# fritzsedlazeck/Sniffles

Measured on NVIDIA H100. Metric: aligned long-read Gbp/s through lead->cluster->consensus, higher is better.
Workload: dtype int32

## Files before the change

sniffles_b200/csrc/api.cu:

```cuda
#include <algorithm>
#include <climits>
#include <cstdio>
#include <cstdlib>
#include <cstring>
#include <string>
#include <vector>
#include <dlfcn.h>
#include <omp.h>

#include "common.cuh"
#include "prims.cuh"
#include "extract.cuh"
#include "cluster.cuh"
#include "consensus.cuh"
#include "poa.cuh"
#include "combine.cuh"
#include "ingest.cuh"
#include "bgzf_write.cuh"

template <bool Pinned> struct Buf {
    void* p = nullptr; size_t cap = 0;
    Buf() = default;
    Buf(const Buf&) = delete; Buf& operator=(const Buf&) = delete;
    ~Buf() { release(); }
// ... 213 lines not shown
    for (int i = 0; i <= MAX_TIMINGS; ++i) cudaEventDestroy(ctx->ev[i]);
    cudaEventDestroy(ctx->ev_b); cudaEventDestroy(ctx->ev_mid); cudaEventDestroy(ctx->ev_fork); cudaEventDestroy(ctx->ev_join);
    cudaStreamDestroy(ctx->st_side); cudaStreamDestroy(ctx->st_copy); cudaStreamDestroy(ctx->st);
    delete ctx;
}

const char* snfb_last_error(snfb_ctx* ctx) { return ctx ? ctx->err.c_str() : "null context"; }

int snfb_set_config(snfb_ctx* ctx, const snfb_config* cfg) {
    if (!ctx || !cfg) return 1;
    ctx->force_no_cuts = false;
    if (cfg->consensus_kmer_len != 6) return fail(ctx, "consensus_kmer_len must be 6 (the reference fixes it, config.py:550)");
    if (cfg->cluster_binsize <= 0 || cfg->cluster_resplit_binsize <= 0 || cfg->coverage_binsize <= 0) return fail(ctx, "bin sizes must be positive");
    ctx->cfg = *cfg; ctx->have_cfg = true; ctx->stage_a_done = ctx->stage_b_done = ctx->stage_c_done = false; return 0;
}

static bool c16_offsets(const snfb_rec* rec_in, uint64_t n_rec, const uint32_t* cigar32, std::vector<uint64_t>& off) {
    off.assign(n_rec + 1, 0);
    const uint8_t* raw = reinterpret_cast<const uint8_t*>(cigar32);
    bool bad = false;
    #pragma omp parallel for schedule(static) reduction(|| : bad)
    for (long long i = 0; i < (long long)n_rec; ++i) {
        long long ref; int b = 0;
        const uint32_t w = ingest::c16_convert<1>(raw, 4ull * rec_in[i].cigar_off, rec_in[i].n_cigar, nullptr, 0, 0, &ref, &b);
        bad = bad || b; off[i + 1] = (w + 7) & ~7ull;
    }
    if (bad) return false;
    for (uint64_t i = 0; i < n_rec; ++i) off[i + 1] += off[i];
    return true;
}
static void c16_fill(const snfb_rec* rec_in, uint64_t n_rec, const uint32_t* cigar32, const std::vector<uint64_t>& off, snfb_rec* rec_out, uint16_t* out16, uint32_t evt_min) {
    const uint8_t* raw = reinterpret_cast<const uint8_t*>(cigar32);
    #pragma omp parallel for schedule(static)
    for (long long i = 0; i < (long long)n_rec; ++i) {
        uint16_t* dst = out16 + off[i]; const uint64_t span = off[i + 1] - off[i];
        long long ref; int bad = 0;
        const uint64_t k = ingest::c16_convert<1>(raw, 4ull * rec_in[i].cigar_off, rec_in[i].n_cigar, dst, evt_min, 0, &ref, &bad);
        if (k < span) memset(dst + k, 0, 2 * (span - k));
        snfb_rec r = rec_in[i]; r.n_cigar = (uint32_t)k; r.cigar_off = off[i];
        rec_out[i] = r;
    }
    memset(out16 + off[n_rec], 0, 16);
}
uint64_t snfb_pack_cigar16(const snfb_rec* rec_in, uint64_t n_rec, const uint32_t* cigar32, snfb_rec* rec_out, uint16_t* out16, uint64_t out_cap, uint32_t evt_min) {
    if (n_rec && (!rec_in || !cigar32)) return UINT64_MAX;
    if (evt_min == 0) evt_min = SNFB_CIGAR16_EVT_MIN;
    std::vector<uint64_t> off;
    if (!c16_offsets(rec_in, n_rec, cigar32, off)) return UINT64_MAX;
    const uint64_t total = off[n_rec] + 8;
    if (!out16) return total;
    if (!rec_out || out_cap < total) return UINT64_MAX;
    c16_fill(rec_in, n_rec, cigar32, off, rec_out, out16, evt_min);
    return total;
}

__global__ void k_validate(const snfb_rec* __restrict__ rec, uint32_t n_rec, uint32_t n_task, uint64_t n_cigar, uint64_t n_var, uint64_t n_seq, int check_seq, DevCounters* ctr) {
    const uint32_t i = blockIdx.x * blockDim.x + threadIdx.x; if (i >= n_rec) return;
    const snfb_rec r = rec[i];
    bool bad = r.task < 0 || (uint32_t)r.task >= n_task || (r.cigar_off & 7) || r.cigar_off + (uint64_t)r.n_cigar > n_cigar || r.var_off + (uint64_t)r.l_qname + r.sa_len > n_var || r.l_seq < 0;
    if (check_seq && r.l_seq >= 0 && r.seq_off + (uint64_t)((r.l_seq + 1) / 2) > n_seq) bad = true;
    if (bad) atomicAdd(&ctr->bad_records, 1ULL);
}

static int check_tables(snfb_ctx* ctx, const snfb_records* R) {
    for (uint32_t t = 0; t < R->n_task; ++t) {
        const snfb_task& k = R->task[t];
        if (k.tr_n < 0 || k.tr_off < 0 || (uint64_t)k.tr_off + (uint64_t)k.tr_n > R->n_tr) return fail(ctx, "task table: tandem-repeat range outside tr[]");
        if (R->n_contig && (k.contig < 0 || (uint32_t)k.contig >= R->n_contig)) return fail(ctx, "task table: contig index out of range");
        if (k.contig_len < 0 || k.start > k.end) return fail(ctx, "task table: bad region");
        if ((long long)k.contig_len >= ((long long)1 << 26) * (long long)(ctx->have_cfg ? ctx->cfg.cluster_binsize : 100)) return fail(ctx, "contig too long for the bin field of the sort key (contig_len / cluster_binsize must stay below 2^26)");
    }
    if (R->n_mask && R->mask && R->mask_task_off) {
        for (uint32_t t = 0; t < R->n_task; ++t) if (R->mask_task_off[t] > R->mask_task_off[t + 1] || R->mask_task_off[t + 1] > R->n_mask) return fail(ctx, "mask_task_off must be non-decreasing and end at n_mask");
    }
    return 0;
}
static int upload_tables(snfb_ctx* ctx, const snfb_records* R) {
    ctx->tasks.assign(R->task, R->task + R->n_task);
    if (ctx->b_task.ensure(sizeof(snfb_task) * R->n_task) || ctx->b_contig.ensure(sizeof(snfb_contig) * (R->n_contig + 1)) || ctx->b_tr.ensure(8 * ((size_t)R->n_tr + 1)) || ctx->b_trp.ensure(4 * ((size_t)R->n_tr + 1)))
        return fail(ctx, "out of device memory for the task tables");
    CUDA_TRY(cudaMemcpyAsync(ctx->b_task.p, R->task, sizeof(snfb_task) * R->n_task, cudaMemcpyHostToDevice, ctx->st));
    if (R->n_contig) CUDA_TRY(cudaMemcpyAsync(ctx->b_contig.p, R->contig, sizeof(snfb_contig) * R->n_contig, cudaMemcpyHostToDevice, ctx->st));
    if (R->n_tr) {
        std::vector<int32_t> pm(R->n_tr);
        for (uint32_t t = 0; t < R->n_task; ++t) { int32_t m = INT32_MIN; for (int k = 0; k < R->task[t].tr_n; ++k) { const int idx = R->task[t].tr_off + k; if (R->tr[2 * idx + 1] > m) m = R->tr[2 * idx + 1]; pm[idx] = m; } }
        CUDA_TRY(cudaMemcpyAsync(ctx->b_tr.p, R->tr, 8 * (size_t)R->n_tr, cudaMemcpyHostToDevice, ctx->st));
        CUDA_TRY(cudaMemcpyAsync(ctx->b_trp.p, pm.data(), 4 * (size_t)R->n_tr, cudaMemcpyHostToDevice, ctx->st));
        CUDA_TRY(cudaStreamSynchronize(ctx->st));
    }
    ctx->n_mask = (R->mask && R->mask_task_off) ? R->n_mask : 0;
    if (ctx->n_mask) {
        std::vector<uint32_t> mt(ctx->n_mask);
        for (uint32_t t = 0; t < R->n_task; ++t) for (uint32_t m = R->mask_task_off[t]; m < R->mask_task_off[t + 1] && m < ctx->n_mask; ++m) mt[m] = t;
        if (ctx->b_mask.ensure(8 * (size_t)ctx->n_mask) || ctx->b_mask_off.ensure(4 * ((size_t)R->n_task + 1)) || ctx->b_mask_task.ensure(4 * (size_t)ctx->n_mask)) return fail(ctx, "out of device memory (N mask)");
        CUDA_TRY(cudaMemcpyAsync(ctx->b_mask.p, R->mask, 8 * (size_t)ctx->n_mask, cudaMemcpyHostToDevice, ctx->st));
        CUDA_TRY(cudaMemcpyAsync(ctx->b_mask_off.p, R->mask_task_off, 4 * ((size_t)R->n_task + 1), cudaMemcpyHostToDevice, ctx->st));
        CUDA_TRY(cudaMemcpyAsync(ctx->b_mask_task.p, mt.data(), 4 * (size_t)ctx->n_mask, cudaMemcpyHostToDevice, ctx->st));
        CUDA_TRY(cudaStreamSynchronize(ctx->st));
    }
    return 0;
}

int snfb_load_records(snfb_ctx* ctx, const snfb_records* R) {
    if (!ctx || !R) return 1;
    cudaSetDevice(ctx->device);
    ctx->loaded = false; ctx->stage_a_done = ctx->stage_b_done = ctx->stage_c_done = false; ctx->force_no_cuts = false;
    if (R->n_task == 0 || R->n_task > 65535) return fail(ctx, "n_task must be in 1..65535");
    if (R->n_rec >= (1ull << 28)) return fail(ctx, "too many records in one block (2^28)");
    if (!R->task || (R->n_rec && (!R->rec || !R->cigar))) return fail(ctx, "null table in the record block");
    if (check_tables(ctx, R)) return 1;
    ctx->n_rec = R->n_rec; ctx->n_cigar = R->n_cigar; ctx->n_var = R->n_var; ctx->n_seq = R->n_seq;
    ctx->n_task = R->n_task; ctx->n_contig = R->n_contig; ctx->n_tr = R->n_tr; ctx->on_device = R->on_device == SNFB_MEM_DEVICE; ctx->seq_on_demand = R->on_device == SNFB_MEM_HOST_SEQ_ON_DEMAND; ctx->h_seq = ctx->seq_on_demand ? R->seq : nullptr;
    ctx->n_ev = 0;
    const snfb_rec* src_rec = R->rec; const uint16_t* src_cigar = reinterpret_cast<const uint16_t*>(R->cigar); uint64_t n_words = R->n_cigar;
// ... 267 lines not shown
    b.cl_nsub = c.take<uint32_t>(n); b.cl_nvalid = c.take<uint32_t>(n); b.cl_nlead = c.take<uint32_t>(n); b.cl_nrn = c.take<uint32_t>(n); b.cl_cand_base = c.take<uint32_t>(n); b.cl_lead_base = c.take<uint32_t>(n); b.cl_rn_base = c.take<uint32_t>(n);
    ctx->arena_off = c.take<uint32_t>(n);
}
static void carve_c(snfb_ctx* ctx, Carver& c) {
    const Caps& k = ctx->cap; cluster::B& b = ctx->B; consensus::C& cc = ctx->Cc;
    b.cand = c.take<snfb_cand>(k.cand + 1); b.cand_leads = c.take<snfb_lead>(k.cand_lead + 1); b.out_plo = c.take<uint32_t>(k.cand_lead + 1); b.out_pn = c.take<uint32_t>(k.cand_lead + 1);
    b.rnames = c.take<uint64_t>(k.rn + 1); b.rn_off_out = c.take<uint32_t>(k.cand + 2);
    cc.plan_best = c.take<uint32_t>(k.cand + 1); cc.plan_nother = c.take<uint32_t>(k.cand + 1); cc.plan_otot = c.take<uint32_t>(k.cand + 1); cc.alt_len = c.take<uint32_t>(k.cand + 1); cc.scr_len = c.take<uint32_t>(k.cand + 1);
    cc.alt_off = c.take<uint32_t>(k.cand + 1); cc.scr_off = c.take<uint32_t>(k.cand + 1); cc.work_big = c.take<uint32_t>(k.cand + 1); cc.work_small = c.take<uint32_t>(k.cand + 1); cc.work_ctr = c.take<uint32_t>(64);
    cc.items_big = c.take<consensus::C::Item>(k.item + 1); cc.items_small = c.take<consensus::C::Item>(k.item + 1); cc.tiles = c.take<uint2>(k.tile + 1);
    cc.alt = c.take<uint8_t>(k.alt + 64); cc.scr = c.take<uint8_t>(k.scr16 * 16 + 64);
    ctx->seq_req = c.take<consensus::SeqReq>(k.req + 1); ctx->seq_arena = c.take<uint8_t>(k.req16 * 16 + 64);
}
static int ensure_arenas(snfb_ctx* ctx) {
    if (carve(ctx->arena_r, [&](Carver& c) { carve_r(ctx, c); })) return fail(ctx, "out of device memory (per-record arrays)");
    if (carve(ctx->arena_l, [&](Carver& c) { carve_l(ctx, c); })) return fail(ctx, "out of device memory (per-lead arrays)");
    if (carve(ctx->arena_c, [&](Carver& c) { carve_c(ctx, c); })) return fail(ctx, "out of device memory (candidate / consensus arrays)");
    return 0;
}

static void bind_inputs(snfb_ctx* ctx) {
    cluster::B& b = ctx->B;
    b.leads = ctx->leads; b.rec = ctx->d_rec; b.task = ctx->b_task.as<snfb_task>(); b.contig = ctx->b_contig.as<snfb_contig>();
    b.tr = ctx->n_tr ? ctx->b_tr.as<int32_t>() : nullptr; b.tr_pmax = ctx->b_trp.as<int32_t>();
    b.rec_pos = ctx->rec_pos; b.rec_end = ctx->rec_end; b.rec_flags = ctx->rec_flags; b.rec_nm = ctx->rec_nm; b.rec_nlead = ctx->rec_nlead; b.rec_lead_off = ctx->rec_lead_off;
    b.task_first = ctx->task_first; b.task_last = ctx->task_last; b.task_maxspan = ctx->task_span;
    b.mask = ctx->n_mask ? ctx->b_mask.as<int32_t>() : nullptr; b.mask_task_off = ctx->n_mask ? ctx->b_mask_off.as<uint32_t>() : nullptr;
    b.n_task = ctx->n_task; b.n_bound = ctx->cap.lead; b.ctr = ctx->b_ctr.as<DevCounters>(); b.cfg = ctx->cfg;
    b.cut_gap = ctx->force_no_cuts ? INT_MAX : cluster::break_gap(ctx->cfg);
    b.cand_cap = ctx->cap.cand; b.cand_lead_cap = ctx->cap.cand_lead; b.rn_cap = ctx->cap.rn;
    consensus::C& c = ctx->Cc;
    c.cand = b.cand; c.cand_rw = b.cand; c.cand_leads = b.cand_leads; c.out_plo = b.out_plo; c.out_pn = b.out_pn; c.ord = b.ord; c.kleads = b.kleads; c.rec = ctx->d_rec; c.seq = ctx->d_seq; c.arena_off = nullptr;
    c.cand_cap = ctx->cap.cand; c.ctr = b.ctr; c.cfg = ctx->cfg; c.item_cap = ctx->cap.item; c.tile_cap = ctx->cap.tile; c.alt_cap = ctx->cap.alt; c.scr_cap16 = ctx->cap.scr16;
}

static int enqueue_stage_a(snfb_ctx* ctx) {
    const uint64_t nrec = ctx->n_rec; const uint32_t nt = ctx->n_task; const snfb_config& cf = ctx->cfg; cluster::B& b = ctx->B;
    DevCounters* ctr = b.ctr; cudaStream_t st = ctx->st;
    CUDA_TRY(cudaMemsetAsync(ctr, 0, sizeof(DevCounters), st));
    CUDA_TRY(cudaMemsetAsync(ctx->task_first, 0, 4 * nt, st)); CUDA_TRY(cudaMemsetAsync(ctx->task_last, 0, 4 * nt, st));
    CUDA_TRY(cudaMemsetAsync(ctx->task_reads, 0, 4 * nt, st)); CUDA_TRY(cudaMemsetAsync(ctx->task_cov, 0, 8 * nt, st)); CUDA_TRY(cudaMemsetAsync(ctx->task_span, 0, 4 * nt, st));
    CUDA_TRY(cudaMemsetAsync(ctx->task_nm, 0, 8 * nt, st));
    extract::WalkParams S{};
    S.scan = ctx->scanrec; S.n_rec = (uint32_t)nrec; S.cigar = ctx->d_cigar; S.task = b.task;
    S.rec_end = ctx->rec_end; S.rec_nlead = ctx->rec_nlead; S.rec_big = ctx->rec_big;
    S.ev = ctx->ev_buf; S.ev_cap = ctx->cap.lead; S.n_ev = &ctr->n_ev; S.ctr = ctr; S.minsv = cf.minsvlen_screen;
    if (evt_need(ctx) < ctx->evt_min) {
        if (ctx->on_device) return fail(ctx, "the device-resident CIGAR16 arena was packed with a larger event length than the configuration needs: repack with snfb_pack_cigar16(evt_min)");
        launch(ctx->launches, extract::k_reflag, NUM_SMS * 8, 256, 0, st, const_cast<uint16_t*>(ctx->d_cigar), ctx->n_cigar, evt_need(ctx));
        ctx->evt_min = evt_need(ctx);
    }
    mark(ctx, "k_rec_index");
    if (nrec) {
        launch(ctx->launches, k_validate, (unsigned)((nrec + 255) / 256), 256, 0, st, ctx->d_rec, (uint32_t)nrec, nt, ctx->n_cigar, ctx->n_var, ctx->n_seq, ctx->seq_on_demand ? 0 : 1, ctr);
        extract::IndexParams I{};
        I.rec = ctx->d_rec; I.cigar = ctx->d_cigar; I.task = b.task; I.n_rec = (uint32_t)nrec; I.n_task = nt; I.rec_pos = ctx->rec_pos; I.task_first = ctx->task_first; I.task_last = ctx->task_last;
        I.scan = ctx->scanrec; I.clip = ctx->clip; I.rec_end = ctx->rec_end; I.rec_flags = ctx->rec_flags; I.rec_nm = ctx->rec_nm; I.rec_nlead = ctx->rec_nlead; I.ctr = ctr;
        I.mapq_min = cf.mapq; I.alen_min = cf.min_alignment_length; I.excl = cf.exclude_flags; I.want_nm = (cf.qc_nm_measure || cf.phase) ? 1 : 0; I.n_cigar = ctx->n_cigar;
        I.sa_list = ctx->sa_list; I.n_sa = &ctr->n_sa;
        launch(ctx->launches, extract::k_rec_index, (unsigned)((nrec + 255) / 256), 256, 0, st, I);
        mark(ctx, "k_scan", 2 * ctx->n_cigar);
        if (nrec >= extract::WALK_WIDE_MIN) launch(ctx->launches, extract::k_cigar_walk<32>, extract::WALK_BLOCKS, extract::WALK_THREADS, 0, st, S);
        else launch(ctx->launches, extract::k_cigar_walk<1>, extract::WALK_BLOCKS, extract::WALK_THREADS, 0, st, S);
        mark(ctx, "k_rec_post");
        extract::PostParams Q{};
        Q.scan = I.scan; Q.clip = I.clip; Q.task = b.task; Q.n_rec = (uint32_t)nrec; Q.rec_end = ctx->rec_end; Q.rec_big = ctx->rec_big; Q.rec_nm = ctx->rec_nm;
        Q.task_reads = ctx->task_reads; Q.task_cov_bp = ctx->task_cov; Q.task_maxspan = ctx->task_span;
        launch(ctx->launches, extract::k_rec_post, (unsigned)((nrec + 255) / 256), 256, 0, st, Q);
        mark(ctx, "k_emit");
        extract::EmitParams E{};
        E.rec = ctx->d_rec; E.clip = ctx->clip; E.var = ctx->d_var; E.ev = S.ev; E.n_ev = S.n_ev; E.ev_cap = ctx->cap.lead;
        E.leads = ctx->leads; E.ctr = ctr; E.maxlen = cf.dev_seq_cache_maxlen; E.detect_large_ins = cf.detect_large_ins; E.longinslen = (double)cf.long_ins_length / 2.0;
        launch(ctx->launches, extract::k_emit, NUM_SMS * 16, 128, 0, st, E);
        mark(ctx, "k_sa");
        extract::SaParams A{};
        A.rec = ctx->d_rec; A.clip = ctx->clip; A.var = ctx->d_var; A.task = b.task; A.contig = b.contig; A.n_contig = ctx->n_contig;
        A.sa_list = ctx->sa_list; A.n_sa = &ctr->n_sa; A.rec_end = ctx->rec_end; A.rec_nlead = ctx->rec_nlead; A.leads = E.leads; A.lead_cap = ctx->cap.lead; A.ctr = ctr; A.cfg = cf; A.seg_scratch = ctx->sa_seg;
        launch(ctx->launches, extract::k_sa, extract::SA_BLOCKS, extract::SA_THREADS, 0, st, A);
        mark(ctx, "k_task_nm");
        const int cpt = (int)((nrec + extract::NM_CHUNK - 1) / extract::NM_CHUNK);
        launch(ctx->launches, extract::k_nm_partial, dim3(cpt, nt), 256, 0, st, ctx->rec_flags, ctx->rec_nm, ctx->task_first, ctx->task_last, ctx->nm_part, ctx->nm_cnt);
        launch(ctx->launches, extract::k_task_nm, nt, 256, 0, st, ctx->task_first, ctx->task_last, ctx->nm_part, ctx->nm_cnt, cpt, ctx->task_nm);
    }
    mark(ctx, "scan_rec_leads");
    prims::exclusive_scan(ctx->launches, ctx->rec_nlead, ctx->rec_lead_off, ctx->scan_tmp_r, nullptr, nrec, &ctr->n_leads, st);
    const unsigned long long nb = b.n_bound; const int g = grid_for(nb, 256);
    mark(ctx, "sort_leads");
    launch(ctx->launches, cluster::k_scatter_keys, g, 256, 0, st, b);
    prims::RadixTemp rt{ ctx->radix_hist, b.scan_tmp };
    bool first = true;
    prims::radix_sort(ctx->launches, b.key0, b.val0, b.key1, b.val1, rt, &ctr->n_leads, nb, cluster::TASK_SHIFT + bits_for(ctx->n_task), &first, st);
    b.skey = first ? b.key0 : b.key1; b.sval = first ? b.val0 : b.val1;
    mark(ctx, "bins");
    launch(ctx->launches, cluster::k_bin_heads, g, 256, 0, st, b);
    prims::exclusive_scan(ctx->launches, b.flag, b.scan, b.scan_tmp, &ctr->n_leads, nb, &ctr->n_bins, st);
    launch(ctx->launches, cluster::k_bin_build, g, 256, 0, st, b);
    launch(ctx->launches, cluster::k_bin_stats, g, 256, 0, st, b);
    mark(ctx, nullptr);
    CUDA_TRY(cudaGetLastError());
    return 0;
}

static int enqueue_stage_b(snfb_ctx* ctx) {
    cluster::B& b = ctx->B; DevCounters* ctr = b.ctr; cudaStream_t st = ctx->st;
    const unsigned long long nb = b.n_bound; const int g = grid_for(nb, 128);
    mark(ctx, "kept_bins");
    prims::exclusive_scan(ctx->launches, b.bin_nl, b.kl_off, b.scan_tmp, &ctr->n_bins, nb, &ctr->n_kl, st);
    prims::exclusive_scan(ctx->launches, b.bin_nlong, b.kll_off, b.scan_tmp, &ctr->n_bins, nb, &ctr->n_kll, st);
    prims::exclusive_scan(ctx->launches, b.bin_kept, b.kb_idx, b.scan_tmp, &ctr->n_bins, nb, &ctr->n_kbins, st);
    launch(ctx->launches, cluster::k_kbin_build, g, 128, 0, st, b);
    launch(ctx->launches, cluster::k_gather_kept, grid_for(nb, 256), 256, 0, st, b);
// ... 472 lines not shown
```

sniffles_b200/csrc/extract.cuh:

```cuda
#pragma once
#include "common.cuh"
#include "cigar16.h"

namespace extract {

constexpr int MAXSEG = 40;

constexpr uint8_t RF_PASS = 1, RF_HAS_NM = 2;

struct Seg {
    int contig, ref_start, ref_end, qry_start, qry_end;
    int meta;
    int nhint;
    int h_type[2], h_start[2], h_len[2], h_none[2];
    int seq_off, seq_len;
};

__device__ __forceinline__ bool op_adds_read(int op) { return (0x193u >> op) & 1u; }
__device__ __forceinline__ bool op_adds_ref(int op) { return (0x18Du >> op) & 1u; }
__device__ __forceinline__ bool op_is_event(int op) { return (0x016u >> op) & 1u; }

__device__ __forceinline__ void store_lead(snfb_lead* dst, const snfb_lead& l) {
    store16(dst, l);
}
// ... 165 lines not shown
                    const int m = classify_splits_dev(cfg, sg, ne + 1, r.l_seq);
                    for (int i = 0; i < m; ++i) for (int h = 0; h < sg[i].nhint; ++h) {
                        const int mqc = (sg[i].meta >> 8) & 255, mqp = (sg[i > 0 ? i - 1 : 0].meta >> 8) & 255;
                        if (!cfg.dev_keep_lowqual_splits && (mqc < mqp ? mqc : mqp) < cfg.mapq) continue;
                        const int ty = sg[i].h_type[h]; const int hs = sg[i].h_start[h];
                        if (sg[i].contig != tk.contig || hs < tk.start || hs >= tk.end) continue;
                        snfb_lead L;
                        L.rec = rec; L.qname_hash = a.qh; L.read_len = 0; L.seq_off = -1; L.seq_len = 0; L.mate_contig = -1; L.mate_pos = 0; L.nm_sa = 0;
                        L.ref_start = hs; L.ref_end = (!sg[i].h_none[h] && ty != SNFB_INS) ? hs + sg[i].h_len[h] : hs;
                        L.qry_start = sg[i].qry_start; L.qry_end = sg[i].qry_end; L.svlen = sg[i].h_len[h];
                        uint32_t f = (uint32_t)ty | ((uint32_t)((sg[i].meta >> 16) & 3) << 3) | ((sg[i].meta & 1) ? SNFB_LF_REVERSE : 0u) | ((uint32_t)mqc << 16) | ((uint32_t)a.hp << 24);
                        if (sg[i].h_none[h]) f |= SNFB_LF_SVLEN_NONE;
                        if (ty == SNFB_INS && (sg[i].meta & (1 << 20))) { f |= SNFB_LF_HAS_SEQ; L.seq_off = sg[i].seq_off; L.seq_len = sg[i].seq_len; }
                        L.flags = f; L.task = (uint16_t)r.task; L.k = (uint16_t)(a.nlead + added);
                        const unsigned long long slot = alloc_slot_lane(*a.slots, P.leads, P.lead_cap, a.n_slots);
                        if (slot < P.lead_cap) store_lead(P.leads + slot, L); else ++overflow;
                        ++added;
                    }
                }
            }
        }
    }
    *soft_p += soft; *overflow_p += overflow;
    return added;
}


__device__ __forceinline__ void c16_op(const uint32_t (&ww)[4], int h, unsigned& cls, unsigned& len) {
    unsigned x[3];
    #pragma unroll
    for (int e = 0; e < 3; ++e) x[e] = h + e < 8 ? (ww[(h + e) >> 1] >> (16 * ((h + e) & 1))) & 0xffffu : 0u;
    unsigned c = 0, l = 0;
    if (!(x[0] & C16_EXT)) {
        c = c16_word_class(x[0]); l = x[0] & C16_LEN_MASK;
        if (x[1] & C16_EXT) {
            l += c16_ext_add(x[1]);
            if (x[2] & C16_EXT) l += c16_ext_add(x[2]);
        }
    }
    cls = c; len = l;
}
__device__ __forceinline__ void c16_decode8(const uint32_t (&ww)[4], unsigned (&cls)[8], unsigned (&len)[8]) {
    #pragma unroll
    for (int h = 0; h < 8; ++h) c16_op(ww, h, cls[h], len[h]);
}

struct RecScan { uint32_t cig8; uint32_t n_words; int32_t pos; uint32_t meta; };
constexpr int CH = 16;
__host__ __device__ __forceinline__ uint32_t chunks_of(uint32_t n_words) { return (((n_words + 7u) >> 3) + (uint32_t)CH - 1u) / (uint32_t)CH; }
struct RecClip { int32_t alen, qas, clip_left, clip_right; };
constexpr uint32_t RM_PASS = 1u << 24, RM_HAS_NM = 1u << 25, RM_HAS_SA = 1u << 26;

struct IndexParams {
    const snfb_rec* rec; const uint16_t* cigar; const snfb_task* task; uint32_t n_rec; uint32_t n_task; unsigned long long n_cigar;
    int32_t* rec_pos; uint32_t* task_first; uint32_t* task_last;
    RecScan* scan; RecClip* clip; int32_t* rec_end; uint8_t* rec_flags; double* rec_nm; uint32_t* rec_nlead;
    uint32_t* sa_list; unsigned long long* n_sa;
    DevCounters* ctr; int mapq_min, alen_min, excl, want_nm;
};
__device__ __forceinline__ bool index_record(const IndexParams& P, uint32_t i) {
    const uint4* core = reinterpret_cast<const uint4*>(P.rec + i);
    const uint4 c0 = __ldg(core), c1 = __ldg(core + 1), c2 = __ldg(core + 2);
    const int task = (int)c0.x, pos = (int)c0.y; const unsigned flag = c0.z & 0xffffu, mapq = (c0.z >> 16) & 255u, aux = c0.z >> 24; unsigned hp = c0.w & 255u;
    const int nm = (int)c1.x; const uint32_t n = c1.z; const int l_seq = (int)c1.w;
    const unsigned long long cigar_off = (unsigned long long)c2.z | ((unsigned long long)c2.w << 32);
    if ((uint32_t)task >= P.n_task || (cigar_off & 7) || cigar_off + n > P.n_cigar) {
        RecScan s; s.cig8 = 0; s.n_words = 0; s.pos = pos; s.meta = 0; store16(P.scan + i, s);
        RecClip c; c.alen = 0; c.qas = 0; c.clip_left = 0; c.clip_right = 0; store16(P.clip + i, c);
        P.rec_pos[i] = pos; P.rec_flags[i] = 0; P.rec_nm[i] = -1.0; P.rec_end[i] = -1; P.rec_nlead[i] = 0; return false;
    }
    P.rec_pos[i] = pos;
    if (i == 0) P.task_first[task] = 0;
    else { const int2 pv = __ldg(reinterpret_cast<const int2*>(P.rec + i - 1)); if (pv.x != task) { P.task_first[task] = i; if ((uint32_t)pv.x < P.n_task) P.task_last[pv.x] = i; } else if (pv.y > pos) atomicAdd(&P.ctr->unsorted, 1ULL); }
    if (i + 1 == P.n_rec) P.task_last[task] = P.n_rec;
    const uint16_t* cg = P.cigar + cigar_off;
    int qas = 0, qae = l_seq, clip_left = 0, clip_right = 0; uint32_t fe = 0;
    { bool first = true; uint32_t k = 0;
      while (k < n) {
          const unsigned w = __ldg(cg + k); if (w == 0) { ++k; continue; }
          unsigned len = w & C16_LEN_MASK; const unsigned cls = c16_word_class(w); uint32_t k2 = k + 1;
          while (k2 < n) { const unsigned e = __ldg(cg + k2); if (!(e & C16_EXT)) break; len += c16_ext_add(e); ++k2; }
          if (first) { if (cls == C16_S || cls == C16_H) clip_left = (int)len; first = false; fe = k2; }
          if (cls == C16_S) qas += (int)len; else if (cls != C16_H) break;
          k = k2;
      } }
    { bool last = true; long k = (long)n - 1;
      while (k >= (long)fe) {
          long b = k; while (b > (long)fe && (__ldg(cg + b) & C16_EXT)) --b;
          const unsigned w = __ldg(cg + b); if (w == 0) { k = b - 1; continue; }
          unsigned len = w & C16_LEN_MASK; const unsigned cls = c16_word_class(w);
          for (long e2 = b + 1; e2 <= k; ++e2) { const unsigned e = __ldg(cg + e2); len += c16_ext_add(e); }
          if (last) { if (cls == C16_S || cls == C16_H) clip_right = (int)len; last = false; }
          if (cls == C16_S) qae -= (int)len; else if (cls != C16_H) break;
          k = b - 1;
      }
      if (last) clip_right = clip_left; }
    const int alen = qae - qas;
    const snfb_task tk = P.task[task];
    const bool pass = !((int)mapq < P.mapq_min || (flag & 256u) || alen < P.alen_min) && !(P.excl && (flag & (unsigned)P.excl)) && pos >= tk.start && pos < tk.end && n > 0;
    const bool has_nm = pass && P.want_nm && (aux & SNFB_AUX_NM);
    if (!(aux & SNFB_AUX_HP)) hp = 0;
    if (pass && hp > 2) { hp = 0; atomicAdd(&P.ctr->soft_errors, 1ULL); }
    RecScan s; s.cig8 = (uint32_t)(cigar_off >> 3); s.n_words = n; s.pos = pos;
    s.meta = ((uint32_t)task & 0xffffu) | (mapq << 16) | (pass ? RM_PASS : 0u) | (has_nm ? RM_HAS_NM : 0u) | ((pass && (aux & SNFB_AUX_SA)) ? RM_HAS_SA : 0u) | ((pass ? hp : 0u) << 27);
    store16(P.scan + i, s);
    RecClip c; c.alen = alen; c.qas = qas; c.clip_left = clip_left; c.clip_right = clip_right;
    store16(P.clip + i, c);
    P.rec_flags[i] = pass ? (uint8_t)(RF_PASS | (has_nm ? RF_HAS_NM : 0) | (hp << 2)) : (uint8_t)0;
    P.rec_nm[i] = has_nm ? (double)nm : -1.0;
    P.rec_end[i] = -1; P.rec_nlead[i] = 0;
    return pass && (aux & SNFB_AUX_SA);
}
__global__ void __launch_bounds__(256) k_rec_index(const IndexParams P) {
    __shared__ unsigned long long s_base;
    const uint32_t i = blockIdx.x * 256 + threadIdx.x;
    const uint32_t has_sa = i < P.n_rec && index_record(P, i) ? 1u : 0u;
    uint32_t tot; const uint32_t mine = prims::block_excl_scan(has_sa, &tot);
    if (threadIdx.x == 0) s_base = tot ? atomicAdd(P.n_sa, (unsigned long long)tot) : 0ull;
    __syncthreads();
    if (has_sa) P.sa_list[s_base + mine] = i;
}

struct Event { uint32_t rec; uint32_t len; uint32_t pos_q; int32_t pos_r; uint32_t k_cls; uint32_t pad[3]; };

struct WalkParams {
    const RecScan* scan; uint32_t n_rec;
    const uint16_t* cigar; const snfb_task* task;
    int32_t* rec_end; uint32_t* rec_nlead; int32_t* rec_big;
    Event* ev; unsigned long long ev_cap; unsigned long long* n_ev;
    DevCounters* ctr;
    int minsv;
};
constexpr int WALK_THREADS = 256, WALK_BLOCKS = NUM_SMS * 4;
constexpr unsigned long long WALK_WIDE_MIN = 32ull * WALK_BLOCKS * (WALK_THREADS / 32);
constexpr unsigned WALK_SLOTS = 64;

__global__ void k_reflag(uint16_t* __restrict__ cigar, unsigned long long n_words, unsigned evt_min) {
    for (unsigned long long i = blockIdx.x * (unsigned long long)blockDim.x + threadIdx.x; i < n_words; i += (unsigned long long)gridDim.x * blockDim.x) {
        const unsigned w = cigar[i]; if (w & (C16_EXT | C16_E)) continue;
        uint32_t len = w & C16_LEN_MASK;
        if (len < evt_min && (i & 7) != 7 && (cigar[i + 1] & C16_EXT)) len = 1u << C16_LEN_BITS;
        const unsigned e = c16_e_flag(c16_word_class(w), len, evt_min);
        if (e) cigar[i] = (uint16_t)(w | e);
    }
}

__device__ __forceinline__ uint2 lane_sums_ext(uint32_t w0, uint32_t w1, uint32_t w2, uint32_t w3) {
    const uint32_t ww[4] = { w0, w1, w2, w3 };
    unsigned cls[8], len[8]; c16_decode8(ww, cls, len);
// ... 4 lines not shown
}

#define SNFB_WORD_BODY(w, aq, ar) { const uint32_t t_ = (w) >> 11; aq += (w) & ((t_ & 0x00010001u) * 0x7ffu); ar += (w) & (((t_ >> 1) & 0x00010001u) * 0x7ffu); }

__device__ __forceinline__ uint2 group_sums(const uint4 v) {
    if ((v.x | v.y | v.z | v.w) & 0x80008000u) return lane_sums_ext(v.x, v.y, v.z, v.w);
    uint32_t aq = 0, ar = 0;
    SNFB_WORD_BODY(v.x, aq, ar) SNFB_WORD_BODY(v.y, aq, ar) SNFB_WORD_BODY(v.z, aq, ar) SNFB_WORD_BODY(v.w, aq, ar)
    return make_uint2((aq & 0xffffu) + (aq >> 16), (ar & 0xffffu) + (ar >> 16));
}

__device__ __forceinline__ uint32_t seg_incl_sum(uint32_t v, int h, uint32_t init) {
    const uint32_t s = prims::warp_incl_scan(v);
    const uint32_t eh = __shfl_sync(FULL, s - v, h < 0 ? 0 : h);
    return init + s - eh;
}

template <class Emit>
__device__ __forceinline__ void group_events(const uint4 v, uint32_t q0, int r0, int minsv, int tk_start, int tk_end, uint32_t& big, Emit&& emit) {
    const uint32_t ww[4] = { v.x, v.y, v.z, v.w };
    if ((v.x | v.y | v.z | v.w) & 0x80008000u) {
        uint32_t q = q0; int r = r0;
        #pragma unroll
        for (int x = 0; x < 8; ++x) {
            unsigned cls, len; c16_op(ww, x, cls, len);
            if (len > 10u && (cls == C16_I || cls == C16_D)) big += len;
            if (c16_is_event(cls) && (int)len >= minsv) {
                const int rsig = cls == C16_D ? r + (int)len : r;
                if (rsig >= tk_start && rsig < tk_end) emit(cls, len, q, r);
            }
            q += len * (cls & 1u); r += (int)(len * ((cls >> 1) & 1u));
        }
        return;
    }
    uint32_t em = ((v.x >> 14) & 1u) | ((v.x >> 29) & 2u) | ((v.y >> 12) & 4u) | ((v.y >> 27) & 8u)
                | ((v.z >> 10) & 16u) | ((v.z >> 25) & 32u) | ((v.w >> 8) & 64u) | ((v.w >> 23) & 128u);
    for (; em; em &= em - 1u) {
        const uint32_t h = (uint32_t)__ffs(em) - 1u;
        const uint32_t w = h < 4u ? (h < 2u ? v.x : v.y) : (h < 6u ? v.z : v.w);
        const uint32_t x = (w >> (16u * (h & 1u))) & 0xffffu;
        const unsigned cls = c16_word_class(x), len = x & C16_LEN_MASK;
        if (len > 10u && (cls == C16_I || cls == C16_D)) big += len;
        if (!(c16_is_event(cls) && (int)len >= minsv)) continue;
        uint32_t aq = 0, ar = 0;
        #pragma unroll
        for (int i = 0; i < 4; ++i) {
            const uint32_t m = 2u * i + 2u <= h ? 0xffffffffu : (2u * i + 1u == h ? 0xffffu : 0u);
            SNFB_WORD_BODY(ww[i] & m, aq, ar)
        }
        const uint32_t q = q0 + (aq & 0xffffu) + (aq >> 16); const int r = r0 + (int)((ar & 0xffffu) + (ar >> 16));
        const int rsig = cls == C16_D ? r + (int)len : r;
        if (rsig >= tk_start && rsig < tk_end) emit(cls, len, q, r);
    }
}

template <int TILE>
__global__ void __launch_bounds__(WALK_THREADS, 4) k_cigar_walk(const __grid_constant__ WalkParams P) {
    __shared__ uint4 s_rs[WALK_THREADS], s_carry[WALK_THREADS / 32];
    const uint4* __restrict__ cig4 = reinterpret_cast<const uint4*>(P.cigar);
    const uint32_t lane = lane_id();
    uint4* const rs = s_rs + (threadIdx.x & ~31u); uint4& carry = s_carry[threadIdx.x >> 5];
    const uint32_t warp = (blockIdx.x * WALK_THREADS + threadIdx.x) >> 5, n_warps = gridDim.x * (WALK_THREADS / 32);
    unsigned long long s_cur = 0; uint32_t s_left = 0;
    uint32_t run_rec = HOLE, run_cnt = 0;
    uint32_t overflow = 0;
    for (uint32_t t0 = warp * TILE; t0 < P.n_rec; t0 += n_warps * TILE) {
        uint4 d = make_uint4(0u, 0u, 0u, 0u);
        if (lane < (uint32_t)TILE && t0 + lane < P.n_rec) d = __ldg(reinterpret_cast<const uint4*>(P.scan + t0 + lane));
        __syncwarp();
        rs[lane] = d;
        __syncwarp();
        const uint32_t nch = (d.w & RM_PASS) ? chunks_of(d.y) : 0u;
        const uint32_t incl = prims::warp_incl_scan(nch), off = incl - nch, total = __shfl_sync(FULL, incl, 31);
        for (uint32_t c0 = 0; c0 < total; c0 += 32) {
            const uint32_t c = c0 + lane;
            int j = 0;
            #pragma unroll
            for (int s = 16; s; s >>= 1) { const uint32_t o = __shfl_sync(FULL, off, j + s); if (o <= c) j += s; }
            const uint32_t k = c - __shfl_sync(FULL, off, j), G = (rs[j].y + 7u) >> 3;
            const bool valid = c < total, head = valid && k == 0, last = valid && (k + 1u) * CH >= G;
            const int ng = valid ? (int)min((uint32_t)CH, G - k * CH) : 0;
            const uint32_t g0 = rs[j].x + k * CH;
            uint32_t vq = 0, vr = 0, flags = 0;
            {
                const uint4* src = cig4 + g0;
                #pragma unroll 1
                for (int gb = 0; gb < ng; gb += 8) {
                    uint4 v[8];
                    #pragma unroll
                    for (int g = 0; g < 8; ++g) v[g] = gb + g < ng ? __ldg(src + gb + g) : make_uint4(0u, 0u, 0u, 0u);
                    uint32_t aq = 0, ar = 0, ext = 0;
                    #pragma unroll
                    for (int g = 0; g < 8; ++g) {
                        const uint32_t rb = v[g].x | v[g].y | v[g].z | v[g].w;
                        flags |= rb & 0x40004000u;
                        if (rb & 0x80008000u) ext |= 1u << g;
                        else { SNFB_WORD_BODY(v[g].x, aq, ar) SNFB_WORD_BODY(v[g].y, aq, ar) SNFB_WORD_BODY(v[g].z, aq, ar) SNFB_WORD_BODY(v[g].w, aq, ar) }
                    }
                    vq += (aq & 0xffffu) + (aq >> 16); vr += (ar & 0xffffu) + (ar >> 16);
                    for (; ext; ext &= ext - 1u) { const uint4 w = __ldg(src + gb + __ffs(ext) - 1); const uint2 t = lane_sums_ext(w.x, w.y, w.z, w.w); vq += t.x; vr += t.y; }
                }
            }
            const unsigned hm = __ballot_sync(FULL, head) & (lanemask_lt() | (1u << lane));
            const int h = hm ? 31 - __clz(hm) : -1;
            const uint32_t pq = seg_incl_sum(vq, h, h < 0 ? carry.x : 0u) - vq, pr = seg_incl_sum(vr, h, h < 0 ? carry.y : rs[j].z) - vr;
            uint32_t my_n = 0, my_big = 0;
            const uint32_t fng = flags ? (uint32_t)ng : 0u;
            const uint32_t fin = prims::warp_incl_scan(fng), fex = fin - fng, ftot = __shfl_sync(FULL, fin, 31);
            uint32_t cq = 0, cr = 0;
            for (uint32_t p0 = 0; p0 < ftot; p0 += 32) {
                const uint32_t x = p0 + lane;
                const bool gv = x < ftot;
                int o = 0;
                #pragma unroll
                for (int s = 16; s; s >>= 1) { const uint32_t e = __shfl_sync(FULL, fex, o + s); if (e <= x) o += s; }
                const uint32_t gi = x - __shfl_sync(FULL, fex, o), o_g0 = __shfl_sync(FULL, g0, o), o_pq = __shfl_sync(FULL, pq, o), o_pr = __shfl_sync(FULL, pr, o);
                const int o_j = __shfl_sync(FULL, j, o);
                const uint4 v = gv ? __ldg(cig4 + o_g0 + gi) : make_uint4(0u, 0u, 0u, 0u);
                const uint2 a = group_sums(v);
                const unsigned gh = __ballot_sync(FULL, gv && gi == 0) & (lanemask_lt() | (1u << lane));
                const int hg = gh ? 31 - __clz(gh) : -1;
                const uint32_t q = seg_incl_sum(a.x, hg, hg < 0 ? cq : o_pq) - a.x, r = seg_incl_sum(a.y, hg, hg < 0 ? cr : o_pr) - a.y;
                cq = __shfl_sync(FULL, q + a.x, 31); cr = __shfl_sync(FULL, r + a.y, 31);
                const uint32_t f_rec = t0 + (uint32_t)o_j;
                int tk_start = 0, tk_end = 0; uint32_t n = 0, big = 0;
                if (gv && (((v.x | v.y | v.z | v.w) & 0x40004000u) != 0)) {
                    const snfb_task& tk = P.task[rs[o_j].w & 0xffffu];
                    tk_start = tk.start; tk_end = tk.end;
                    group_events(v, q, (int)r, P.minsv, tk_start, tk_end, big, [&](unsigned, unsigned, uint32_t, int) { ++n; });
                }
                const uint32_t n_incl = prims::warp_incl_scan(n), n_ex = n_incl - n, n_tot = __shfl_sync(FULL, n_incl, 31);
                const uint32_t b_incl = prims::warp_incl_scan(big);
                const uint32_t lo = fex > p0 ? fex - p0 : 0u, hi = fin - p0 < 32u ? fin - p0 : 32u;
                const bool mine = fng && fin > p0 && fex < p0 + 32u;
                const uint32_t hi_n = __shfl_sync(FULL, n_incl, (hi - 1u) & 31u), lo_n = __shfl_sync(FULL, n_ex, lo & 31u);
                const uint32_t hi_b = __shfl_sync(FULL, b_incl, (hi - 1u) & 31u), lo_b = __shfl_sync(FULL, b_incl - big, lo & 31u);
                if (mine) { my_n += hi_n - lo_n; my_big += hi_b - lo_b; }
                if (n_tot) {
                    const uint32_t prev_rec = __shfl_up_sync(FULL, f_rec, 1);
                    const unsigned rh = __ballot_sync(FULL, gv && (lane == 0 ? f_rec != run_rec : f_rec != prev_rec)) & (lanemask_lt() | (1u << lane));
                    const int hr = rh ? 31 - __clz(rh) : -1;
                    const uint32_t ord = (hr < 0 ? run_cnt : 0u) + n_ex - __shfl_sync(FULL, n_ex, hr < 0 ? 0 : hr);
                    const uint32_t lastv = ftot - p0 < 32u ? ftot - p0 - 1u : 31u;
// ... 180 lines not shown
```

Measured before the change: 9441.

## Fold record validation into index kernel, read clip ends from two vectors, prefetch CIGAR via L2

Removes the separate k_validate launch and performs the same bounds checks inside k_rec_index, loading one extra 16-byte chunk of the record. Soft/hard-clip detection now reads only the first and last 16-byte CIGAR groups and walks them in registers, falling back to per-word loads when the clip region spans more than those groups. The CIGAR walk loads switch to ld.global.nc with an L2::256B prefetch hint. These changes aim to save a kernel launch, a pass over the record array and scattered 2-byte loads, at the cost of more code complexity and extra prefetch traffic.

```diff
diff --git a/sniffles_b200/csrc/api.cu b/sniffles_b200/csrc/api.cu
--- a/sniffles_b200/csrc/api.cu
+++ b/sniffles_b200/csrc/api.cu
@@ -289,14 +289,6 @@
     if (!rec_out || out_cap < total) return UINT64_MAX;
     c16_fill(rec_in, n_rec, cigar32, off, rec_out, out16, evt_min);
     return total;
-}
-
-__global__ void k_validate(const snfb_rec* __restrict__ rec, uint32_t n_rec, uint32_t n_task, uint64_t n_cigar, uint64_t n_var, uint64_t n_seq, int check_seq, DevCounters* ctr) {
-    const uint32_t i = blockIdx.x * blockDim.x + threadIdx.x; if (i >= n_rec) return;
-    const snfb_rec r = rec[i];
-    bool bad = r.task < 0 || (uint32_t)r.task >= n_task || (r.cigar_off & 7) || r.cigar_off + (uint64_t)r.n_cigar > n_cigar || r.var_off + (uint64_t)r.l_qname + r.sa_len > n_var || r.l_seq < 0;
-    if (check_seq && r.l_seq >= 0 && r.seq_off + (uint64_t)((r.l_seq + 1) / 2) > n_seq) bad = true;
-    if (bad) atomicAdd(&ctr->bad_records, 1ULL);
 }
 
 static int check_tables(snfb_ctx* ctx, const snfb_records* R) {
@@ -670,11 +662,11 @@
     }
     mark(ctx, "k_rec_index");
     if (nrec) {
-        launch(ctx->launches, k_validate, (unsigned)((nrec + 255) / 256), 256, 0, st, ctx->d_rec, (uint32_t)nrec, nt, ctx->n_cigar, ctx->n_var, ctx->n_seq, ctx->seq_on_demand ? 0 : 1, ctr);
         extract::IndexParams I{};
         I.rec = ctx->d_rec; I.cigar = ctx->d_cigar; I.task = b.task; I.n_rec = (uint32_t)nrec; I.n_task = nt; I.rec_pos = ctx->rec_pos; I.task_first = ctx->task_first; I.task_last = ctx->task_last;
         I.scan = ctx->scanrec; I.clip = ctx->clip; I.rec_end = ctx->rec_end; I.rec_flags = ctx->rec_flags; I.rec_nm = ctx->rec_nm; I.rec_nlead = ctx->rec_nlead; I.ctr = ctr;
-        I.mapq_min = cf.mapq; I.alen_min = cf.min_alignment_length; I.excl = cf.exclude_flags; I.want_nm = (cf.qc_nm_measure || cf.phase) ? 1 : 0; I.n_cigar = ctx->n_cigar;
+        I.mapq_min = cf.mapq; I.alen_min = cf.min_alignment_length; I.excl = cf.exclude_flags; I.want_nm = (cf.qc_nm_measure || cf.phase) ? 1 : 0;
+        I.n_cigar = ctx->n_cigar; I.n_var = ctx->n_var; I.n_seq = ctx->n_seq; I.check_seq = ctx->seq_on_demand ? 0 : 1;
         I.sa_list = ctx->sa_list; I.n_sa = &ctr->n_sa;
         launch(ctx->launches, extract::k_rec_index, (unsigned)((nrec + 255) / 256), 256, 0, st, I);
         mark(ctx, "k_scan", 2 * ctx->n_cigar);
diff --git a/sniffles_b200/csrc/extract.cuh b/sniffles_b200/csrc/extract.cuh
--- a/sniffles_b200/csrc/extract.cuh
+++ b/sniffles_b200/csrc/extract.cuh
@@ -241,49 +241,77 @@
 constexpr uint32_t RM_PASS = 1u << 24, RM_HAS_NM = 1u << 25, RM_HAS_SA = 1u << 26;
 
 struct IndexParams {
-    const snfb_rec* rec; const uint16_t* cigar; const snfb_task* task; uint32_t n_rec; uint32_t n_task; unsigned long long n_cigar;
+    const snfb_rec* rec; const uint16_t* cigar; const snfb_task* task; uint32_t n_rec; uint32_t n_task; unsigned long long n_cigar, n_var, n_seq;
+    int check_seq;
     int32_t* rec_pos; uint32_t* task_first; uint32_t* task_last;
     RecScan* scan; RecClip* clip; int32_t* rec_end; uint8_t* rec_flags; double* rec_nm; uint32_t* rec_nlead;
     uint32_t* sa_list; unsigned long long* n_sa;
     DevCounters* ctr; int mapq_min, alen_min, excl, want_nm;
 };
-__device__ __forceinline__ bool index_record(const IndexParams& P, uint32_t i) {
-    const uint4* core = reinterpret_cast<const uint4*>(P.rec + i);
-    const uint4 c0 = __ldg(core), c1 = __ldg(core + 1), c2 = __ldg(core + 2);
-    const int task = (int)c0.x, pos = (int)c0.y; const unsigned flag = c0.z & 0xffffu, mapq = (c0.z >> 16) & 255u, aux = c0.z >> 24; unsigned hp = c0.w & 255u;
-    const int nm = (int)c1.x; const uint32_t n = c1.z; const int l_seq = (int)c1.w;
-    const unsigned long long cigar_off = (unsigned long long)c2.z | ((unsigned long long)c2.w << 32);
-    if ((uint32_t)task >= P.n_task || (cigar_off & 7) || cigar_off + n > P.n_cigar) {
-        RecScan s; s.cig8 = 0; s.n_words = 0; s.pos = pos; s.meta = 0; store16(P.scan + i, s);
-        RecClip c; c.alen = 0; c.qas = 0; c.clip_left = 0; c.clip_right = 0; store16(P.clip + i, c);
-        P.rec_pos[i] = pos; P.rec_flags[i] = 0; P.rec_nm[i] = -1.0; P.rec_end[i] = -1; P.rec_nlead[i] = 0; return false;
-    }
-    P.rec_pos[i] = pos;
-    if (i == 0) P.task_first[task] = 0;
-    else { const int2 pv = __ldg(reinterpret_cast<const int2*>(P.rec + i - 1)); if (pv.x != task) { P.task_first[task] = i; if ((uint32_t)pv.x < P.n_task) P.task_last[pv.x] = i; } else if (pv.y > pos) atomicAdd(&P.ctr->unsorted, 1ULL); }
-    if (i + 1 == P.n_rec) P.task_last[task] = P.n_rec;
-    const uint16_t* cg = P.cigar + cigar_off;
-    int qas = 0, qae = l_seq, clip_left = 0, clip_right = 0; uint32_t fe = 0;
+
+template <class Word>
+__device__ __forceinline__ void clip_walk(uint32_t n, Word&& word, int& qas, int& qae, int& clip_left, int& clip_right) {
+    uint32_t fe = 0;
     { bool first = true; uint32_t k = 0;
       while (k < n) {
-          const unsigned w = __ldg(cg + k); if (w == 0) { ++k; continue; }
+          const unsigned w = word(k); if (w == 0) { ++k; continue; }
           unsigned len = w & C16_LEN_MASK; const unsigned cls = c16_word_class(w); uint32_t k2 = k + 1;
-          while (k2 < n) { const unsigned e = __ldg(cg + k2); if (!(e & C16_EXT)) break; len += c16_ext_add(e); ++k2; }
+          while (k2 < n) { const unsigned e = word(k2); if (!(e & C16_EXT)) break; len += c16_ext_add(e); ++k2; }
           if (first) { if (cls == C16_S || cls == C16_H) clip_left = (int)len; first = false; fe = k2; }
           if (cls == C16_S) qas += (int)len; else if (cls != C16_H) break;
           k = k2;
       } }
     { bool last = true; long k = (long)n - 1;
       while (k >= (long)fe) {
-          long b = k; while (b > (long)fe && (__ldg(cg + b) & C16_EXT)) --b;
-          const unsigned w = __ldg(cg + b); if (w == 0) { k = b - 1; continue; }
+          long b = k; while (b > (long)fe && (word((uint32_t)b) & C16_EXT)) --b;
+          const unsigned w = word((uint32_t)b); if (w == 0) { k = b - 1; continue; }
           unsigned len = w & C16_LEN_MASK; const unsigned cls = c16_word_class(w);
-          for (long e2 = b + 1; e2 <= k; ++e2) { const unsigned e = __ldg(cg + e2); len += c16_ext_add(e); }
+          for (long e2 = b + 1; e2 <= k; ++e2) len += c16_ext_add(word((uint32_t)e2));
           if (last) { if (cls == C16_S || cls == C16_H) clip_right = (int)len; last = false; }
           if (cls == C16_S) qae -= (int)len; else if (cls != C16_H) break;
           k = b - 1;
       }
       if (last) clip_right = clip_left; }
+}
+__device__ __forceinline__ unsigned end_word(const uint4& f, const uint4& l, uint32_t l0, uint32_t k, bool& miss) {
+    const bool in_f = k < 8u, in_l = k >= l0;
+    if (!in_f && !in_l) miss = true;
+    const uint4 v = in_f ? f : l; const uint32_t h = (k & 7u) >> 1;
+    const uint32_t x = h < 2u ? (h ? v.y : v.x) : (h == 2u ? v.z : v.w);
+    return (in_f || in_l) ? (x >> (16u * (k & 1u))) & 0xffffu : C16_M << C16_CLASS_SHIFT;
+}
+
+__device__ __forceinline__ bool index_record(const IndexParams& P, uint32_t i) {
+    const uint4* core = reinterpret_cast<const uint4*>(P.rec + i);
+    const uint4 c0 = __ldg(core), c1 = __ldg(core + 1), c2 = __ldg(core + 2), c3 = __ldg(core + 3);
+    const int task = (int)c0.x, pos = (int)c0.y; const unsigned flag = c0.z & 0xffffu, mapq = (c0.z >> 16) & 255u, aux = c0.z >> 24; unsigned hp = c0.w & 255u;
+    const uint32_t l_qname = (c0.w >> 8) & 255u;
+    const int nm = (int)c1.x; const uint32_t n = c1.z; const int l_seq = (int)c1.w; const uint32_t sa_len = c2.x;
+    const unsigned long long cigar_off = (unsigned long long)c2.z | ((unsigned long long)c2.w << 32);
+    const unsigned long long seq_off = (unsigned long long)c3.x | ((unsigned long long)c3.y << 32), var_off = (unsigned long long)c3.z | ((unsigned long long)c3.w << 32);
+    const bool bad_core = (uint32_t)task >= P.n_task || (cigar_off & 7) || cigar_off + n > P.n_cigar;
+    const bool bad = bad_core || var_off + l_qname + sa_len > P.n_var || l_seq < 0
+                     || (P.check_seq && seq_off + (unsigned long long)((l_seq + 1) / 2) > P.n_seq);
+    if (bad) atomicAdd(&P.ctr->bad_records, 1ULL);
+    if (bad_core) {
+        RecScan s; s.cig8 = 0; s.n_words = 0; s.pos = pos; s.meta = 0; store16(P.scan + i, s);
+        RecClip c; c.alen = 0; c.qas = 0; c.clip_left = 0; c.clip_right = 0; store16(P.clip + i, c);
+        P.rec_pos[i] = pos; P.rec_flags[i] = 0; P.rec_nm[i] = -1.0; P.rec_end[i] = -1; P.rec_nlead[i] = 0; return false;
+    }
+    P.rec_pos[i] = pos;
+    if (i == 0) P.task_first[task] = 0;
+    else { const int2 pv = __ldg(reinterpret_cast<const int2*>(P.rec + i - 1)); if (pv.x != task) { P.task_first[task] = i; if ((uint32_t)pv.x < P.n_task) P.task_last[pv.x] = i; } else if (pv.y > pos) atomicAdd(&P.ctr->unsorted, 1ULL); }
+    if (i + 1 == P.n_rec) P.task_last[task] = P.n_rec;
+    const uint16_t* cg = P.cigar + cigar_off;
+    int qas = 0, qae = l_seq, clip_left = 0, clip_right = 0;
+    const uint32_t G = (n + 7u) >> 3;
+    bool miss = G == 0 || cigar_off + 8ull * G > P.n_cigar;
+    if (!miss) {
+        const uint4* g4 = reinterpret_cast<const uint4*>(cg);
+        const uint4 f = __ldg(g4), l = __ldg(g4 + (G - 1u)); const uint32_t l0 = 8u * (G - 1u);
+        clip_walk(n, [&](uint32_t k) { return end_word(f, l, l0, k, miss); }, qas, qae, clip_left, clip_right);
+    }
+    if (miss) { qas = 0; qae = l_seq; clip_left = 0; clip_right = 0; clip_walk(n, [&](uint32_t k) { return (unsigned)__ldg(cg + k); }, qas, qae, clip_left, clip_right); }
     const int alen = qae - qas;
     const snfb_task tk = P.task[task];
     const bool pass = !((int)mapq < P.mapq_min || (flag & 256u) || alen < P.alen_min) && !(P.excl && (flag & (unsigned)P.excl)) && pos >= tk.start && pos < tk.end && n > 0;
@@ -394,6 +422,10 @@
         const int rsig = cls == C16_D ? r + (int)len : r;
         if (rsig >= tk_start && rsig < tk_end) emit(cls, len, q, r);
     }
+}
+
+__device__ __forceinline__ uint4 ldg_l2_256(const uint4* p) {
+    uint4 v; asm("ld.global.nc.L2::256B.v4.u32 {%0, %1, %2, %3}, [%4];" : "=r"(v.x), "=r"(v.y), "=r"(v.z), "=r"(v.w) : "l"(p)); return v;
 }
 
 template <int TILE>
@@ -430,7 +462,7 @@
                 for (int gb = 0; gb < ng; gb += 8) {
                     uint4 v[8];
                     #pragma unroll
-                    for (int g = 0; g < 8; ++g) v[g] = gb + g < ng ? __ldg(src + gb + g) : make_uint4(0u, 0u, 0u, 0u);
+                    for (int g = 0; g < 8; ++g) v[g] = gb + g < ng ? ldg_l2_256(src + gb + g) : make_uint4(0u, 0u, 0u, 0u);
                     uint32_t aq = 0, ar = 0, ext = 0;
                     #pragma unroll
                     for (int g = 0; g < 8; ++g) {
```

Measured after the change: 9824 (median of 6 runs). 4.1% higher.
